# Arktis2022/Spiking-Diffusion

Hardware: AMD Instinct MI355X
Metric: images/sec + LIF-kernel HBM GB/s, MNIST 100-step sample T=16, 1->8 GPU (higher is better)
Workload: dtype fp32-exact (4 fp6 digits x fp4 spikes on the block-scaled MFMA + certified decisions + exact 6-digit recomputation of flagged neurons)

## Files before the change

### spiking-diffusion_amd/csrc/den_mfma_fp6v2.hip

```cpp
#include "cert_common.h"
#include "../../include/spkdiff.h"
#include <stdlib.h>
#include <type_traits>
#include <utility>

namespace {

constexpr int CK = 32;
constexpr int N_PAIR = 18;
constexpr int N_D4 = 5;
constexpr int N_MAIN = N_PAIR + N_D4;
constexpr int N_L5 = 2;
constexpr int NACC = 2;
constexpr int W_PIECES = (N_PAIR * WT + 1023) / 1024;
constexpr int W_LDS = W_PIECES * 1024;
constexpr int W_SLAB = ((N_MAIN + N_L5) * WT + 1023) / 1024 * 1024;

struct V2Args {
  const uint8_t* in0; int nch;
  const uint8_t* wq; const double* scale; const double* bias; const float* wl1;
  const float* bn_a; const float* bn_b;
  uint8_t* out; uint8_t* out_cnt;
  CertWs ws;
  int handover;
  const int* qtab;
  const int* n_dyn;
  const uint8_t* need; const int* cls_cnt; const int* cls_list;
  int B, Cout, Cin;
  int gx, nsets;
};

constexpr int SPK_V2_KMIN = 2;
constexpr float SPK_V2_SPARE = 1.0f;
constexpr int SPK_V2_REC_STEP = 13;
constexpr int SPK_V2_LP_PAIRS = 1;
constexpr int SPK_V2_GX_KB = 2560;
constexpr int SPK_V2_HALF_FILL = 2;
constexpr int SPK_V2_LPS_MIN_B = 64;
constexpr int SPK_V2_LP_SPLIT_MAX = 512;
constexpr int SPK_V2_PF = 6;


__device__ __forceinline__ void store_tile_spikes(uint8_t* out, uint8_t* out_cnt, unsigned mybits, int lane, long long rec_base,
                                                  long long cnt_base, bool ok) {
  const unsigned bitsv = spk_transpose16_rows(mybits, lane);
  if (out_cnt && ok) out_cnt[cnt_base + (lane & 31)] = (uint8_t)__popc(mybits);
  if (ok) *reinterpret_cast<uint2*>(out + rec_base + (lane & 15) * 16 + 8 * ((lane >> 4) & 1)) = spk_e2m1_record(bitsv);
}

__device__ const uint8_t V2_HALF_REC[2][64] = {
    {0, 1, 2, 3, 4, 5, 6, 7, 8, 9, 10, 11, 12, 13, 14, 15, 16, 17, 18, 19, 20, 21, 22, 23,
     23, 23, 23, 23, 23, 23, 23, 23, 23, 23, 23, 23, 23, 23, 23, 23, 23, 23, 23, 23, 23, 23, 23, 23, 24},
    {24, 25, 26, 27, 28, 29, 30, 31, 32, 33, 34, 35, 36, 37, 38, 39, 40, 41, 42, 43, 44, 45, 46, 47,
     47, 47, 47, 47, 47, 47, 47, 47, 47, 47, 47, 47, 47, 47, 47, 47, 47, 47, 47, 47, 47, 47, 47, 47, 24}};

enum : int { V2_INT = 0, V2_TOP, V2_RIGHT, V2_LEFT, V2_BOTTOM, V2_NCLS };
struct V2Plan { int nblk; int tap[9]; int nt[9]; };
constexpr int V2_FT = 3;
constexpr V2Plan V2_PLAN[V2_NCLS] = {
    {9, {0, 1, 2, 3, 4, 5, 6, 7, 8}, {3, 3, 3, 3, 3, 3, 3, 3, 3}},
    {6, {3, 4, 5, 6, 7, 8}, {3, 3, 3, 3, 3, 3}},
    {6, {0, 1, 3, 4, 6, 7}, {3, 3, 3, 3, 3, 3}},
    {6, {1, 2, 4, 5, 7, 8}, {3, 3, 3, 3, 3, 3}},
    {9, {0, 6, 7, 8, 1, 2, 3, 4, 5}, {3, 1, 1, 1, 3, 3, 3, 3, 3}}};
constexpr V2Plan v2_uniform_plan(int nt) {
  V2Plan p = {9, {0, 1, 2, 3, 4, 5, 6, 7, 8}, {}};
  for (int b = 0; b < 9; ++b) p.nt[b] = nt;
  return p;
}
constexpr int v2_plan_start(const V2Plan& p, int blk) {
  int n = 0;
  for (int b = 0; b < blk; ++b) n += p.nt[b];
  return n;
}
constexpr int v2_plan_blk(const V2Plan& p, int s) {
  int b = 0;
  while (s >= p.nt[b]) s -= p.nt[b++];
  return b;
}
__device__ constexpr uint8_t V2_FULL_POS[8][V2_FT][2] = {
    {{0, 1}, {2, 3}, {4, 5}},       {{6, 13}, {20, 27}, {34, 41}},  {{7, 14}, {21, 28}, {35, 42}},  {{43, 44}, {45, 46}, {47, 40}},
    {{8, 9}, {10, 11}, {12, 15}},   {{16, 17}, {18, 19}, {22, 23}}, {{24, 25}, {26, 29}, {30, 31}}, {{32, 33}, {36, 37}, {38, 39}}};
__device__ constexpr uint8_t V2_WAVE_CLS[8] = {V2_TOP, V2_RIGHT, V2_LEFT, V2_BOTTOM, V2_INT, V2_INT, V2_INT, V2_INT};
constexpr bool v2_full_map_ok() {
  bool seen[48] = {};
  for (int w = 0; w < 8; ++w)
    for (int i = 0; i < V2_FT; ++i)
      for (int h = 0; h < 2; ++h) {
        const int p = V2_FULL_POS[w][i][h];
        if (p >= 48 || seen[p]) return false;
        seen[p] = true;
      }
  for (int w = 0; w < 8; ++w) {
    const V2Plan& pl = V2_PLAN[V2_WAVE_CLS[w]];
    for (int i = 0; i < V2_FT; ++i)
      for (int tap = 0; tap < 9; ++tap) {
        int n = 0;
        for (int b = 0; b < pl.nblk; ++b) n += pl.tap[b] == tap && i >= V2_FT - pl.nt[b];
        if (n > 1) return false;
        for (int h = 0; h < 2 && n == 0; ++h) {
          const int y = V2_FULL_POS[w][i][h] / 7 + tap / 3 - 1, x = V2_FULL_POS[w][i][h] % 7 + tap % 3 - 1;
          if (y >= 0 && y < 7 && x >= 0 && x < 7) return false;
        }
      }
  }
  return true;
}
static_assert(v2_full_map_ok(), "full 7x7 items: position table and block lists");

constexpr int V2_FULL_NCA = 3, V2_FULL_NCWW = 3;
constexpr int v2_ceil_div(int a, int b) { return (a + b - 1) / b; }
constexpr int v2_copy_na(int na, int ncw, int w) {
  const int npa = v2_ceil_div(na, ncw), left = na - w * npa;
  return w >= ncw || left <= 0 ? 0 : (left < npa ? left : npa);
}
constexpr int v2_copy_nw(int nw, int ncw, int w) {
  return w >= ncw || w >= nw ? 0 : (nw - w + ncw - 1) / ncw;
}
constexpr int v2_rec_off(int r, int nrec, int w) {
  const int cl = r >> 4, t = r & 15;
  return r < nrec ? (((cl / w) + 1) * (w + 1) + 1 + (cl % w)) * POSB + t * 16 : 0;
}
constexpr bool v2_roles_ok(int nwv, int nca, int ncww, int na, int nw, int nrec, int w) {
  int pa[64] = {}, pw[64] = {};
  if (na > 64 || nw > 64 || nca > nwv || ncww > nwv) return false;
  for (int wv = 0; wv < nwv; ++wv) {
    for (int j = 0; j < v2_copy_na(na, nca, wv); ++j) ++pa[wv * v2_ceil_div(na, nca) + j];
    for (int q = 0; q < v2_copy_nw(nw, ncww, wv); ++q) ++pw[wv + ncww * q];
  }
  for (int i = 0; i < na; ++i) if (pa[i] != 1) return false;
  for (int i = 0; i < nw; ++i) if (pw[i] != 1) return false;
  const int nct = 64 * nwv, nr = v2_ceil_div(nrec, nct);
  int seen[1024] = {};
  if (nrec > 1024) return false;
  for (int tid = 0; tid < nct; ++tid)
    for (int k = 0; k < nr; ++k) {
      const int r = tid + k * nct, off = v2_rec_off(r, nrec, w);
      if (r < nrec) {
        const int cell = off / POSB, y = cell / (w + 1), x = cell % (w + 1);
        if (y < 1 || x < 1 || x > w || (y - 1) * w + (x - 1) != (r >> 4) || (off % POSB) != (r & 15) * 16) return false;
        ++seen[r];
      } else if (off != 0) return false;
    }
  for (int r = 0; r < nrec; ++r) if (seen[r] != 1) return false;
  return true;
}
static_assert(v2_roles_ok(8, V2_FULL_NCA, V2_FULL_NCWW, 7 * 2, W_PIECES, 7 * 7 * 16, 7), "full 7x7 items: 41 pieces, 784 records, one owner each");

template <int H, int W, int NWV, bool SPLIT, int NTP, bool HALF = false, int CLS = V2_INT>
__device__ __forceinline__ void fp6v2_body(const V2Args& a, const int g, const int il, const int lanes, const int n_images,
                                           const int* __restrict__ slots, const int n_live = 0) {
  constexpr bool PRUNE = NTP > 0;
  constexpr bool LIVE = PRUNE && !HALF;
  static_assert(!HALF || (PRUNE && !SPLIT && H == 7 && W == 7 && NWV == 4 && NTP == 3), "half-image items: 7x7, four waves x three tiles");
  constexpr bool REC = !PRUNE;
  constexpr int HW = H * W, PW = W + 1;
  constexpr int Hb = SPLIT ? H / 2 : H;
  constexpr int Hin = SPLIT ? Hb + 1 : H;
  constexpr int HWb = Hb * W;
  static_assert(SPLIT ? ((H % 2) == 0 && (HWb % (2 * NWV)) == 0)
                      : ((HW & 1) == 1 && ((HW / 2) % NWV) == 0), "whole 32-row tiles on every wave (+ one odd position)");
  static_assert(!PRUNE || (!SPLIT && (NWV == 4 || NWV == 8) && NTP <= (HWb / 2) / NWV), "position lists: 7x7 items");
  constexpr int NT = PRUNE ? NTP : (HWb / 2) / NWV;
  constexpr int N_AGPR = NWV == 4 ? (NACC * NT < 16 ? NACC * NT : 16) : 0;
  constexpr int NPP = (Hin + 2) * PW + 1;
  constexpr int A_BYTES = NPP * POSB;
  constexpr int PPR = (W + 3) / 4;
  constexpr int NA = Hin * PPR;
  constexpr bool BSKIP = NWV == 8 && !PRUNE && !SPLIT;
  static_assert(!BSKIP || (H == 7 && W == 7 && NT == V2_FT), "border skip: the position table is for 7x7 items of three tiles per wave");
  static_assert(BSKIP || CLS == V2_INT, "wave classes: full 7x7 items only");
  constexpr int NCA = BSKIP ? V2_FULL_NCA : NWV, NCWW = BSKIP ? V2_FULL_NCWW : NWV;
  constexpr bool KNOWN = BSKIP && CLS != V2_INT;
  constexpr int CWV = KNOWN ? CLS - 1 : 0;
  static_assert(!KNOWN || V2_WAVE_CLS[CWV] == CLS, "border class k is wave k - 1");
  static_assert(!BSKIP || v2_roles_ok(NWV, NCA, NCWW, NA, W_PIECES, Hin * W * 16, W), "copy roles, record counting");
  constexpr int NPA_T = (NA + NCA - 1) / NCA;
  constexpr int NPA = KNOWN ? v2_copy_na(NA, NCA, CWV) : ((!BSKIP || NCA == NWV) ? NPA_T : 0);
  constexpr int NPW = KNOWN ? v2_copy_nw(W_PIECES, NCWW, CWV) : ((!BSKIP || NCWW == NWV) ? (W_PIECES + NCWW - 1) / NCWW : 0);
  static_assert(NWV >= 8 || NACC * NT <= 16 || (NT - 1) * NACC <= N_AGPR + 2, "only the last tile may straddle the register files");
  constexpr bool AH = NWV == 8 && !PRUNE;
  constexpr int NBUF = 2;
  extern __shared__ __attribute__((aligned(16))) uint8_t lds[];
  uint8_t* const sA = lds;
  uint8_t* const sW = lds + NBUF * A_BYTES;
  int* const s_cin = reinterpret_cast<int*>(lds + NBUF * A_BYTES + NBUF * W_LDS);
  int* const s_row = s_cin + NPP * 16;
  int* const s_nmax = s_row + (HWb + 1) * 16;
  const unsigned sA_addr = spk_lds_addr(sA), sW_addr = sA_addr + NBUF * A_BYTES;
  const int tid = threadIdx.x, lane = tid & 63, wave = tid >> 6;
  const int nch = a.nch;
  const int G = a.Cout >> 5;
  const int wave_s = KNOWN ? CWV : __builtin_amdgcn_readfirstlane(wave);
  const unsigned lane16 = (unsigned)lane * 16u;
  const unsigned wave_k = (unsigned)wave_s * 1024u;
  const uint8_t* const wbase = a.wq + (long long)g * nch * W_SLAB;
  const int nitems = (SPLIT || HALF) ? 2 * n_images : n_images;
  auto issue_w = [&](int qw, const uint8_t* wslab, unsigned dW) {
    unsigned ko = wave_k + 1024u * NCWW * (unsigned)qw;
    if (NCWW * qw + NCWW - 1 >= W_PIECES) ko = ko < (unsigned)W_PIECES * 1024u ? ko : ko - 1024u * NCWW;
    spk_dma16s(wslab + ko, lane16, dW + ko);
  };
  if constexpr (BSKIP && NPW > 0) {
    if (il < nitems) {
#pragma unroll
      for (int q = 0; q < NPW; ++q) issue_w(q, wbase, sW_addr);
    }
  }
  for (int i = tid; i < NBUF * A_BYTES / 16; i += NWV * 64) reinterpret_cast<uint4*>(sA)[i] = make_uint4(0, 0, 0, 0);
  if (REC)
    for (int i = tid; i < NPP * 16; i += NWV * 64) s_cin[i] = 0;
  __syncthreads();

  const int row = lane & 31, half = lane >> 5;
  const int hsel = (row >> 2) & 1, tt = (row & 3) + 4 * (row >> 3);
  int a_off[NT];
  int p_out[NT];
#pragma unroll
  for (int i = 0; i < NT; ++i) {
    const int p = BSKIP ? (int)V2_FULL_POS[wave & 7][i % V2_FT][hsel] : 2 * (wave + NWV * i) + hsel;
    a_off[i] = ((p / W) * PW + (p % W)) * POSB + tt * 16;
    p_out[i] = BSKIP ? (int)V2_FULL_POS[wave & 7][i % V2_FT][half] : 2 * (wave + NWV * i) + half;
  }

  unsigned pa_pk[NPA > 0 ? NPA : 1];
#pragma unroll
  for (int j = 0; j < NPA; ++j) {
    int id = wave_s * NPA_T + j;
    id = id < NA ? id : NA - 1;
    const int y = id / PPR, px = id - y * PPR;
    const int np = (W - 4 * px) < 4 ? (W - 4 * px) : 4;
    const unsigned src = (unsigned)((y * W + 4 * px) * POSB), dst = (unsigned)(((y + 1) * PW + 1 + 4 * px) * POSB);
    pa_pk[j] = src | (dst << 14) | ((unsigned)(np - 1) << 29);
  }
  auto issue_piece = [&](int q, const uint8_t* aslab, const uint8_t* wslab, unsigned dA, unsigned dW) {
    if (q < NPA) {
      const unsigned pk = pa_pk[q];
      const unsigned np = ((pk >> 29) & 3u) + 1u;
      const unsigned long long mask = np == 4 ? ~0ull : ((1ull << (16 * np)) - 1ull);
      spk_dma16s_masked(aslab + (pk & 0x3fffu), lane16, dA + ((pk >> 14) & 0x7fffu), mask);
    } else issue_w(q - NPA, wslab, dW);
  };
  auto aslab_of = [&](int itm, int c) -> const uint8_t* {
    const int b = HALF ? itm >> 1 : (PRUNE ? slots[itm] : (SPLIT ? itm >> 1 : itm)), band = SPLIT ? itm & 1 : 0;
    return a.in0 + ((long long)b * nch + c) * HW * POSB + band * (Hb - 1) * W * POSB;
  };

  const int co = g * 32 + (lane & 31);
  const float scale_f = (float)a.scale[co], bias_f = (float)a.bias[co];
  const float bna = a.bn_a[co], bnb = a.bn_b[co];
  const float Bc = fmaf(bias_f, bna, bnb);
  const float cE = 2.0f * 2.38418579e-07f * (fabsf(bnb) + fabsf(Bc)) + 1e-30f;
  const float cT = 528.0f * scale_f * fabsf(bna) * 1.000001f;
  const float Ac4 = 1024.0f * scale_f * bna;

  const int sc_a = 0x7f7f7f7f;
  const int sc_p = half ? (int)0x82828282u : (int)0x87878787u;

  int it = 0;
  if (il < nitems) {
    const uint8_t* as0 = aslab_of(il, 0);
#pragma unroll
    for (int q = 0; q < (BSKIP ? NPA : NPA + NPW); ++q) issue_piece(q, as0, wbase, sA_addr, sW_addr);
    if constexpr (AH) {
      spk_dma_wait_all();
      __syncthreads();
    }
  }
  for (int itm = il; itm < nitems; itm += lanes) {
    const int b = HALF ? itm >> 1 : (PRUNE ? slots[itm] : (SPLIT ? itm >> 1 : itm)), band = SPLIT ? itm & 1 : 0;
    const int band_off = band * PW * POSB;
    int n_list = 2 * NT * NWV;
    if constexpr (PRUNE) {
      const uint8_t* rec = HALF ? &V2_HALF_REC[itm & 1][0] : a.need + (long long)b * 64;
      n_list = __builtin_amdgcn_readfirstlane((int)rec[48]);
#pragma unroll
      for (int i = 0; i < NT; ++i) {
        const int k2 = 2 * (wave + NWV * i);
        const int p = rec[k2 + hsel];
        a_off[i] = ((p / W) * PW + (p % W)) * POSB + tt * 16;
        p_out[i] = rec[k2 + half];
      }
    }
    v16f acc[NT][NACC];
    int cnt[NT];
#pragma unroll
    for (int i = 0; i < NT; ++i) cnt[i] = 0;
    constexpr int NREC = Hin * W * 16, NR = (NREC + NWV * 64 - 1) / (NWV * 64);
    int creg[NR];
    int rec_off[NR];
    bool rec_ok[NR];
#pragma unroll
    for (int k = 0; k < NR; ++k) {
      creg[k] = 0;
      const int r = tid + k * NWV * 64;
      rec_ok[k] = r < NREC;
      rec_off[k] = v2_rec_off(r, NREC, W);
    }
    constexpr int PFX = NWV == 4 ? SPK_V2_PF : 4;
    v6i bp[2][2];
    v4i af[PFX];
    for (int c = 0; c < nch; ++c, ++it) {
      const int buf = it & 1, buf1 = buf ^ 1;
      if constexpr (!AH) {
        spk_dma_wait_all();
        __syncthreads();
      }
      int nb = itm, nc = c + 1;
      if (nc == nch) { nc = 0; nb = itm + lanes; }
      const bool have_next = nb < nitems;
      const uint8_t* n_aslab = aslab_of(have_next ? nb : itm, have_next ? nc : c);
      const uint8_t* n_wslab = wbase + (long long)(have_next ? nc : c) * W_SLAB;
      const unsigned n_dA = sA_addr + buf1 * A_BYTES;
      const unsigned n_dW = sW_addr + buf1 * W_LDS;

      v4i rvq[NR];
      auto compute = [&](auto first_tag) {
        constexpr bool FIRST = decltype(first_tag)::value;
        const uint8_t* A = sA + buf * A_BYTES + band_off;
        const uint8_t* Wb = sW + buf * W_LDS;
        auto toff = [](int tap) constexpr -> int { return ((tap / 3) * PW + (tap % 3)) * POSB; };
        constexpr V2Plan P = BSKIP ? V2_PLAN[CLS] : v2_uniform_plan(NT);
        constexpr int NBLK = P.nblk, NSTEP = v2_plan_start(P, NBLK);
        constexpr int PF = PFX;
        constexpr int NPIECES = NPA + NPW;
        static_assert(P.nt[0] == NT, "the first block writes (not accumulates) every accumulator");
        constexpr bool SLOT1 = BSKIP && (NCA != NWV || NCWW != NWV);
        static_assert(SLOT1 || 2 * NBLK >= NPIECES, "two copy slots per block: every DMA piece of the wave gets one");
        static_assert((!AH || NSTEP >= 2 * PF) && (!REC || NSTEP > SPK_V2_REC_STEP), "look-ahead slots; the record-count steps exist");
        static_assert(!AH || ((SLOT1 ? NPIECES : v2_plan_start(P, (NPIECES + 1) / 2)) <= NSTEP - PF && v2_plan_start(P, NBLK - 2) <= NSTEP - PF),
                      "chunk barrier behind the copies and the last weight-tile read");
        auto lda_at = [&](const uint8_t* base, auto s_tag) -> v4i {
          constexpr int s = decltype(s_tag)::value;
          constexpr int blk = v2_plan_blk(P, s), i = NT - P.nt[blk] + (s - v2_plan_start(P, blk));
          return *reinterpret_cast<const v4i*>(base + a_off[i] + toff(P.tap[blk]));
        };
        auto lda = [&](auto s_tag) -> v4i { return lda_at(A, s_tag); };
        auto ldb = [&](int tile) -> v6i {
          const uint8_t* p = Wb + tile * WT;
          const v4i x = *reinterpret_cast<const v4i*>(p + lane * 16);
          typedef const volatile __attribute__((address_space(3))) v2i* lds_v2i_ptr;
          const v2i y = *(lds_v2i_ptr)SPK_LDS(p + 1024 + lane * 8);
          const v6i r = {x[0], x[1], x[2], x[3], y[0], y[1]};
          return r;
        };
        if constexpr (!AH || FIRST) {
          bp[0][0] = ldb(2 * P.tap[0]); bp[0][1] = ldb(2 * P.tap[0] + 1);
          static_for<PF>([&](auto s_tag) { af[decltype(s_tag)::value] = lda(s_tag); });
        }
        const uint8_t* An = sA + buf1 * A_BYTES + band_off;
        const uint8_t* Wn = sW + buf1 * W_LDS;
        const bool ahead = AH && c + 1 < nch;
        static_for<NSTEP>([&](auto s_tag) {
          constexpr int s = decltype(s_tag)::value;
          constexpr int blk = v2_plan_blk(P, s), nt = P.nt[blk], j = s - v2_plan_start(P, blk);
          constexpr int i = NT - nt + j;
          if constexpr (AH && s == NSTEP - PF) {
            asm volatile("s_waitcnt vmcnt(0)\n\ts_barrier" ::: "memory");
          }
          const v4i av = af[s % PF];
          if constexpr (s + PF < NSTEP) af[s % PF] = lda(std::integral_constant<int, s + PF>{});
          else if constexpr (AH) {
            constexpr int k = s % PF;
            if (ahead) af[k] = lda_at(An, std::integral_constant<int, k>{});
          }
#define V2_DMA_SLOT()                                                                              \
  do {                                                                                             \
    if constexpr (SLOT1 && s < NPIECES) issue_piece(s, n_aslab, n_wslab, n_dA, n_dW);                 \
    if constexpr (!SLOT1 && j == 0 && 2 * blk < NPIECES) issue_piece(2 * blk, n_aslab, n_wslab, n_dA, n_dW);     \
    if constexpr (!SLOT1 && j == (nt > 1 ? nt / 2 : 0) && 2 * blk + 1 < NPIECES)                   \
      issue_piece(2 * blk + 1, n_aslab, n_wslab, n_dA, n_dW);                                      \
  } while (0)
#define V2_NEXT_TILES()                                                                            \
  do {                                                                                             \
    if constexpr (j == 0 && blk + 1 < NBLK) {                                                      \
      bp[(blk + 1) & 1][0] = ldb(2 * P.tap[(blk + 1) % 9]);                                        \
      bp[(blk + 1) & 1][1] = ldb(2 * P.tap[(blk + 1) % 9] + 1);                                    \
    }                                                                                              \
  } while (0)
          if constexpr (!REC) {
            asm volatile("v_bcnt_u32_b32 %0, %1, %0\n\tv_bcnt_u32_b32 %0, %2, %0\n\tv_bcnt_u32_b32 %0, %3, %0\n\t"
                         "v_bcnt_u32_b32 %0, %4, %0" : "+v"(cnt[i]) : "v"(av[0]), "v"(av[1]), "v"(av[2]), "v"(av[3]));
          }
#define V2_PAIR_MFMA(J)                                                                                      \
do {                                                                                                        \
  if constexpr (FIRST && blk == 0) {                                                                        \
    if constexpr (NACC * i + (J) < N_AGPR) SPK_MFMA_FP6_Z("a", acc[i][J], av, bp[0][J], sc_a, sc_p);              \
    else SPK_MFMA_FP6_Z("v", acc[i][J], av, bp[0][J], sc_a, sc_p);                                             \
  } else {                                                                                                  \
    if constexpr (NACC * i + (J) < N_AGPR) SPK_MFMA_FP6("a", acc[i][J], av, bp[blk & 1][J], sc_a, sc_p);          \
    else SPK_MFMA_FP6("v", acc[i][J], av, bp[blk & 1][J], sc_a, sc_p);                                         \
  }                                                                                                         \
} while (0)
          V2_PAIR_MFMA(0);
          __builtin_amdgcn_sched_barrier(0);
          V2_DMA_SLOT();
          V2_NEXT_TILES();
          if constexpr (REC) {
            if constexpr (s == 1) {
#pragma unroll
              for (int k = 0; k < NR; ++k) rvq[k] = *reinterpret_cast<const v4i*>(sA + buf * A_BYTES + rec_off[k]);
            }
            if constexpr (s == SPK_V2_REC_STEP) {
#pragma unroll
              for (int k = 0; k < NR; ++k)
                creg[k] += __builtin_popcount((unsigned)rvq[k][0]) + __builtin_popcount((unsigned)rvq[k][1]) +
                           __builtin_popcount((unsigned)rvq[k][2]) + __builtin_popcount((unsigned)rvq[k][3]);
            }
          }
          V2_PAIR_MFMA(1);
          __builtin_amdgcn_sched_barrier(0);
          if constexpr (AH && s == NSTEP - 1) {
            if (ahead) {
              auto ldb_n = [&](int tile) -> v6i {
                const uint8_t* p = Wn + tile * WT;
                const v4i x = *reinterpret_cast<const v4i*>(p + lane * 16);
                typedef const volatile __attribute__((address_space(3))) v2i* lds_v2i_ptr;
                const v2i y = *(lds_v2i_ptr)SPK_LDS(p + 1024 + lane * 8);
                const v6i r = {x[0], x[1], x[2], x[3], y[0], y[1]};
                return r;
              };
              bp[0][0] = ldb_n(2 * P.tap[0]); bp[0][1] = ldb_n(2 * P.tap[0] + 1);
            }
          }
        });
      };
      if (c == 0) compute(std::true_type{}); else compute(std::false_type{});
    }

    if constexpr (REC) {
#pragma unroll
      for (int k = 0; k < NR; ++k)
        if (rec_ok[k]) s_cin[(rec_off[k] / POSB) * 16 + ((rec_off[k] % POSB) >> 4)] = creg[k];
      if (tid <= HWb) s_nmax[tid] = 0;
      __syncthreads();
      for (int e = tid; e < HWb * 16; e += NWV * 64) {
        const int pp = e >> 4, t = e & 15;
        const int* c0 = s_cin + (((pp / W) + band) * PW + (pp % W)) * 16 + t;
        int sum = 0;
#pragma unroll
        for (int dy = 0; dy < 3; ++dy)
#pragma unroll
          for (int dx = 0; dx < 3; ++dx) sum += c0[(dy * PW + dx) * 16];
        s_row[e] = sum;
        atomicMax(&s_nmax[pp], sum);
      }
      __syncthreads();
    }
    asm volatile("s_nop 15\n\ts_nop 15" ::: "memory");

#pragma unroll
    for (int k = 0; k < NT; ++k) {
      const int i = k == 0 ? NT - 1 : k - 1;
#pragma unroll
      for (int j = 0; j < NACC; ++j)
        if (NACC * i + j < N_AGPR) asm volatile("" : "+a"(acc[i][j]));
      float v = 0.f;
      unsigned mybits = 0;
      bool flg = false;
      int cntv[16];
      if constexpr (!REC) {
#pragma unroll
        for (int r = 0; r < 16; ++r) {
          const int rowA = spk_acc_row(r, 0);
          const int c0 = __builtin_amdgcn_readlane(cnt[i], rowA), c1 = __builtin_amdgcn_readlane(cnt[i], rowA + 4);
          cntv[r] = half ? c1 : c0;
        }
      }
      int nmax_rec = 0;
      if constexpr (REC) nmax_rec = s_nmax[BSKIP ? p_out[i] : 2 * (wave + NWV * i) + half];
      float zmax = 0.f, dmin = 3.0e38f;
      int nmax = nmax_rec;
#pragma unroll
      for (int r2 = 0; r2 < 16; r2 += 2) {
        const v2f p0 = {acc[i][0][r2], acc[i][0][r2 + 1]}, p1 = {acc[i][1][r2], acc[i][1][r2 + 1]};
        const v2f q4 = __builtin_elementwise_fma(p0, (v2f){1024.0f, 1024.0f}, p1);
        const v2f z2 = __builtin_elementwise_fma(q4, (v2f){Ac4, Ac4}, (v2f){Bc, Bc});
        if constexpr (!REC) nmax = max(nmax, max(cntv[r2], cntv[r2 + 1]));
#pragma unroll
        for (int e = 0; e < 2; ++e) {
          const float z = z2[e];
          zmax = fmaxf(zmax, fabsf(z));
          const float h = fmaf(z - v, 0.5f, v);
          const float hm = h - 1.0f;
          dmin = fminf(dmin, fabsf(hm));
          const bool s = h >= 1.0f;
          v = s ? 0.0f : h;
          mybits = __builtin_amdgcn_alignbit(mybits, __float_as_uint(hm), 31);
        }
      }
      mybits = ~(__builtin_bitreverse32(mybits) >> 16) & 0xffffu;
      flg = dmin <= SPK_V2_SPARE * fmaf(zmax, 2.5f * CERT_4EPS, fmaf((float)nmax, cT, cE));
      if (__builtin_amdgcn_ballot_w64(flg) != 0ull) {
        float v2 = 0.f, dh = 0.f;
        bool f2 = false;
        if constexpr (REC) {
          const v4i* rp = reinterpret_cast<const v4i*>(s_row + (BSKIP ? p_out[i] : 2 * (wave + NWV * i) + half) * 16);
#pragma unroll
          for (int q = 0; q < 4; ++q) {
            const v4i c4 = rp[q];
            cntv[4 * q] = c4[0]; cntv[4 * q + 1] = c4[1]; cntv[4 * q + 2] = c4[2]; cntv[4 * q + 3] = c4[3];
          }
        }
#pragma unroll
        for (int r2 = 0; r2 < 16; r2 += 2) {
          const v2f p0 = {acc[i][0][r2], acc[i][0][r2 + 1]}, p1 = {acc[i][1][r2], acc[i][1][r2 + 1]};
          const v2f q4 = __builtin_elementwise_fma(p0, (v2f){1024.0f, 1024.0f}, p1);
          const v2f z2 = __builtin_elementwise_fma(q4, (v2f){Ac4, Ac4}, (v2f){Bc, Bc});
#pragma unroll
          for (int e = 0; e < 2; ++e) {
            const float z = z2[e];
            const float ct = fmaf((float)cntv[r2 + e], cT, cE);
            dh = fmaf(fabsf(z) + fabsf(v2), 0.625f * CERT_4EPS, fmaf(dh, 0.5f, 0.5f * ct));
            const float h = fmaf(z - v2, 0.5f, v2);
            f2 = f2 || (fabsf(h - 1.0f) <= SPK_V2_SPARE * dh);
            v2 = h >= 1.0f ? 0.0f : h;
          }
        }
        flg = flg && f2;
      }
      const int ti = wave + NWV * i;
      const int p = (PRUNE || BSKIP) ? p_out[i] : 2 * ti + half + band * HWb;
      const bool listed = (!PRUNE || 2 * ti + half < n_list) && (!LIVE || b < n_live);
      if (flg && listed) spk_cert_flag(a.ws, ((long long)b * a.Cout + co) * HW + p);
      const long long rec = (((long long)b * G + g) * HW + p) * POSB;
      store_tile_spikes(a.out, a.out_cnt, mybits, lane, rec, (((long long)b * G + g) * HW + p) * 32, listed);
      __builtin_amdgcn_sched_barrier(0);
    }
  }
  spk_dma_wait_all();
}

__device__ __forceinline__ void fp6v2_wg_map(const V2Args& a, int& g, int& il, int& lanes) {
  const int k = blockIdx.x, G = a.Cout >> 5;
  if (a.gx > 0) {
    const int S = gridDim.x >> 3, x = k & 7, slot = k >> 3;
    const int npart = 8 / a.nsets, set = x % a.nsets, xi = x / a.nsets, lanes_x = S / a.gx;
    g = set * a.gx + slot % a.gx;
    il = xi * lanes_x + slot / a.gx;
    lanes = npart * lanes_x;
  } else {
    g = k % G;
    il = k / G;
    lanes = gridDim.x / G;
  }
}

__device__ __forceinline__ void fp6v2_handover(const V2Args& a) {
  if (!a.handover) return;
  __syncthreads();
  if (threadIdx.x == 0) spk_cert_handover(a.ws);
}

template <int H, int W, int NWV, bool SPLIT = false>
__global__ __launch_bounds__(NWV * 64, 1) void conv3x3_fp6v2_kernel(V2Args a) {
  const int Bn = spk_batch_count(a.n_dyn, a.B);
  int g, il, lanes;
  fp6v2_wg_map(a, g, il, lanes);
  if constexpr (NWV == 8 && !SPLIT) {
    switch (__builtin_amdgcn_readfirstlane((int)V2_WAVE_CLS[(threadIdx.x >> 6) & 7])) {
      case V2_TOP: fp6v2_body<H, W, NWV, false, 0, false, V2_TOP>(a, g, il, lanes, Bn, nullptr); break;
      case V2_RIGHT: fp6v2_body<H, W, NWV, false, 0, false, V2_RIGHT>(a, g, il, lanes, Bn, nullptr); break;
      case V2_LEFT: fp6v2_body<H, W, NWV, false, 0, false, V2_LEFT>(a, g, il, lanes, Bn, nullptr); break;
      case V2_BOTTOM: fp6v2_body<H, W, NWV, false, 0, false, V2_BOTTOM>(a, g, il, lanes, Bn, nullptr); break;
      default: fp6v2_body<H, W, NWV, false, 0, false, V2_INT>(a, g, il, lanes, Bn, nullptr); break;
    }
  } else fp6v2_body<H, W, NWV, SPLIT, 0>(a, g, il, lanes, Bn, nullptr);
  fp6v2_handover(a);
}

template <int H, int W>
__global__ __launch_bounds__(256, 1) void conv3x3_fp6v2_half_kernel(V2Args a) {
  const int Bn = spk_batch_count(a.n_dyn, a.B);
  int g, il, lanes;
  fp6v2_wg_map(a, g, il, lanes);
  fp6v2_body<H, W, 4, false, 3, true>(a, g, il, lanes, Bn, nullptr);
  fp6v2_handover(a);
}

template <int H, int W, int NWV>
__global__ __launch_bounds__(NWV * 64, 1) void conv3x3_fp6v2_listed_kernel(V2Args a) {
  constexpr int NC = (H * W / 2) / 4;
  const int Bn = spk_batch_count(a.n_dyn, a.B);
  int g, il, lanes;
  fp6v2_wg_map(a, g, il, lanes);
  int cnt[NC], work[NC], u[NC];
  int total = 0, nonempty = 0;
#pragma unroll
  for (int k = 0; k < NC; ++k) {
    cnt[k] = a.cls_cnt[k];
    work[k] = cnt[k] * (k + 1 < SPK_V2_KMIN ? SPK_V2_KMIN : k + 1);
    total += work[k];
    nonempty += cnt[k] > 0;
  }
  if (total == 0) { fp6v2_handover(a); return; }
  int rem = lanes - nonempty, used = 0;
#pragma unroll
  for (int k = 0; k < NC; ++k) {
    u[k] = cnt[k] > 0 ? 1 + (int)((long long)rem * work[k] / total) : 0;
    used += u[k];
  }
  for (int left = lanes - used; left > 0; --left) {
    int best = 0;
    long long bw = -1, bu = 1;
#pragma unroll
    for (int k = 0; k < NC; ++k)
      if (cnt[k] > 0 && (long long)work[k] * bu > bw * u[k]) { bw = work[k]; bu = u[k]; best = k; }
#pragma unroll
    for (int k = 0; k < NC; ++k) u[k] += (k == best);
  }
  int start = 0, cls = -1, il_c = 0, lanes_c = 1;
#pragma unroll
  for (int k = 0; k < NC; ++k) {
    if (il >= start && il < start + u[k]) { cls = k; il_c = il - start; lanes_c = u[k]; }
    start += u[k];
  }
  const int* slots = a.cls_list + (long long)(cls < 0 ? 0 : cls) * a.B;
  static_assert(NWV == 8, "listed positions: two waves per SIMD");
  switch (cls) {
    case 0: case 1: fp6v2_body<H, W, 8, false, 1>(a, g, il_c, lanes_c, cnt[cls], slots, Bn); break;
    case 2: case 3: fp6v2_body<H, W, 8, false, 2>(a, g, il_c, lanes_c, cnt[cls], slots, Bn); break;
    case 4: case 5: fp6v2_body<H, W, 8, false, 3>(a, g, il_c, lanes_c, cnt[cls], slots, Bn); break;
    default: break;
  }
  fp6v2_handover(a);
}


template <int H, int W, bool WIDE>
__device__ __forceinline__ void fp6v2_lastpos_body(const V2Args& a, const int bid, float (*red)[16][64]) {
  constexpr int HW = H * W, NP = SPK_V2_LP_PAIRS;
  const int lane = threadIdx.x & 63, wave = threadIdx.x >> 6;
  const int nch = a.nch, G = a.Cout >> 5;
  const int Bn = spk_batch_count(a.n_dyn, a.B);
  if (!a.handover && bid == 0 && threadIdx.x == 0) { a.ws.flags[1] = a.ws.flags[0]; a.ws.flags[0] = 0u; }
  const int n_units = ((Bn + 2 * NP - 1) / (2 * NP)) * G;
  const bool split = n_units <= SPK_V2_LP_SPLIT_MAX;
  const int unit = split ? bid : bid * 4 + wave;
  const int g = unit % G, b0 = (unit / G) * 2 * NP;
  if (b0 >= Bn) return;
  const int row = lane & 31, half = lane >> 5;
  const int hsel = (row >> 2) & 1, tt = (row & 3) + 4 * (row >> 3);
  const int sc_a = 0x7f7f7f7f;
  const int sc_p = half ? (int)0x82828282u : (int)0x87878787u;
  const int sc_hi = (int)0x87878787u, sc_lo = (int)0x82828282u;
  v16f acc[NP][3];
#pragma unroll
  for (int q = 0; q < NP; ++q)
#pragma unroll
    for (int j = 0; j < 3; ++j)
#pragma unroll
      for (int r = 0; r < 16; ++r) acc[q][j][r] = 0.f;
  const int py = H - 1, px = W - 1;
  for (int c = split ? wave : 0; c < nch; c += split ? 4 : 1) {
    const uint8_t* wslab = a.wq + ((long long)g * nch + c) * W_SLAB;
    auto ldb = [&](int tile) -> v8i {
      const uint8_t* wt = wslab + tile * WT;
      const v4i bx = *reinterpret_cast<const v4i*>(wt + lane * 16);
      const v2i by = *reinterpret_cast<const v2i*>(wt + 1024 + lane * 8);
      return v8i{bx[0], bx[1], bx[2], bx[3], by[0], by[1], 0, 0};
    };
    v4i sp[NP][4];
#pragma unroll
    for (int q = 0; q < NP; ++q) {
      const int bA = b0 + 2 * q + hsel;
#pragma unroll
      for (int u = 0; u < 4; ++u) {
        const int tap = (u >> 1) * 3 + (u & 1);
        const int yy = py + tap / 3 - 1, xx = px + tap % 3 - 1;
        sp[q][u] = v4i{0, 0, 0, 0};
        if (bA < Bn)
          sp[q][u] = *reinterpret_cast<const v4i*>(a.in0 + (((long long)bA * nch + c) * HW + yy * W + xx) * POSB + tt * 16);
      }
// ... 454 lines not shown
```

Before: 3361.

## Pair adjacent conv taps per MFMA block with compile-time register-slot schedule

For the block-skip (full 7x7) path, adjacent 3x3 taps are grouped into pair blocks so each block covers two taps. The two half-waves read different tap offsets and the weight tiles use interleaved high/low scale selectors, which roughly halves the number of block iterations. A constexpr scheduler places each A and B LDS read a fixed distance ahead of its MFMA, bounded by when its register slot frees up and by the chunk barrier, and static_asserts check that placement. DMA pieces and record-count ops are moved into fixed slots. This adds heavy template complexity and changes register pressure and the scale encoding, which could break exactness if the pairing is wrong.

```diff
diff --git a/spiking-diffusion_amd/csrc/den_mfma_fp6v2.hip b/spiking-diffusion_amd/csrc/den_mfma_fp6v2.hip
--- a/spiking-diffusion_amd/csrc/den_mfma_fp6v2.hip
+++ b/spiking-diffusion_amd/csrc/den_mfma_fp6v2.hip
@@ -39,6 +39,10 @@
 constexpr int SPK_V2_LPS_MIN_B = 64;
 constexpr int SPK_V2_LP_SPLIT_MAX = 512;
 constexpr int SPK_V2_PF = 6;
+constexpr int SPK_V2_TP_SLOTS_INT = 5;
+constexpr int v2_tp_slots(int cls) { return cls == 0 ? SPK_V2_TP_SLOTS_INT : (cls == 4 ? 4 : 3); }
+constexpr int SPK_V2_TP_PFD = 12;
+constexpr int SPK_V2_TP_TAIL = 6;
 
 
 __device__ __forceinline__ void store_tile_spikes(uint8_t* out, uint8_t* out_cnt, unsigned mybits, int lane, long long rec_base,
@@ -55,16 +59,16 @@
      47, 47, 47, 47, 47, 47, 47, 47, 47, 47, 47, 47, 47, 47, 47, 47, 47, 47, 47, 47, 47, 47, 47, 47, 24}};
 
 enum : int { V2_INT = 0, V2_TOP, V2_RIGHT, V2_LEFT, V2_BOTTOM, V2_NCLS };
-struct V2Plan { int nblk; int tap[9]; int nt[9]; };
+struct V2Plan { int nblk; int tap[9]; int nt[9]; int pair[9]; };
 constexpr int V2_FT = 3;
 constexpr V2Plan V2_PLAN[V2_NCLS] = {
-    {9, {0, 1, 2, 3, 4, 5, 6, 7, 8}, {3, 3, 3, 3, 3, 3, 3, 3, 3}},
-    {6, {3, 4, 5, 6, 7, 8}, {3, 3, 3, 3, 3, 3}},
-    {6, {0, 1, 3, 4, 6, 7}, {3, 3, 3, 3, 3, 3}},
-    {6, {1, 2, 4, 5, 7, 8}, {3, 3, 3, 3, 3, 3}},
-    {9, {0, 6, 7, 8, 1, 2, 3, 4, 5}, {3, 1, 1, 1, 3, 3, 3, 3, 3}}};
+    {5, {0, 2, 4, 6, 8}, {3, 3, 3, 3, 3}, {1, 1, 1, 1, 0}},
+    {3, {3, 5, 7}, {3, 3, 3}, {1, 1, 1}},
+    {3, {0, 3, 6}, {3, 3, 3}, {1, 1, 1}},
+    {3, {1, 4, 7}, {3, 3, 3}, {1, 1, 1}},
+    {5, {0, 6, 8, 2, 4}, {3, 1, 1, 3, 3}, {1, 1, 0, 1, 1}}};
 constexpr V2Plan v2_uniform_plan(int nt) {
-  V2Plan p = {9, {0, 1, 2, 3, 4, 5, 6, 7, 8}, {}};
+  V2Plan p = {9, {0, 1, 2, 3, 4, 5, 6, 7, 8}, {}, {}};
   for (int b = 0; b < 9; ++b) p.nt[b] = nt;
   return p;
 }
@@ -77,6 +81,73 @@
   int b = 0;
   while (s >= p.nt[b]) s -= p.nt[b++];
   return b;
+}
+constexpr bool v2_plan_has(const V2Plan& p, int b, int tap) { return p.tap[b] == tap || (p.pair[b] && p.tap[b] + 1 == tap); }
+constexpr int v2p_nd(const V2Plan& p, int b) { return p.pair[b] ? 4 : 2; }
+constexpr int v2p_op_start(const V2Plan& p, int blk) {
+  int n = 0;
+  for (int b = 0; b < blk; ++b) n += v2p_nd(p, b) * p.nt[b];
+  return n;
+}
+constexpr int v2p_op_blk(const V2Plan& p, int m) {
+  int b = 0;
+  while (m >= v2p_op_start(p, b + 1)) ++b;
+  return b;
+}
+constexpr int v2p_swap(int q) { return ((q & 1) << 1) | (q >> 1); }
+constexpr int v2p_op_sel(const V2Plan& p, int b, int q) { return p.nt[b] > 1 ? q / p.nt[b] : (p.pair[b] ? v2p_swap(q) : q); }
+constexpr int v2p_op_tile(const V2Plan& p, int b, int q) { return V2_FT - p.nt[b] + (p.nt[b] > 1 ? q % p.nt[b] : 0); }
+constexpr int v2p_b_start(const V2Plan& p, int blk) {
+  int n = 0;
+  for (int b = 0; b < blk; ++b) n += v2p_nd(p, b);
+  return n;
+}
+constexpr int v2p_b_blk(const V2Plan& p, int g) {
+  int b = 0;
+  while (g >= v2p_b_start(p, b + 1)) ++b;
+  return b;
+}
+constexpr int v2p_a_first(const V2Plan& p, int f) { return v2p_op_start(p, v2_plan_blk(p, f)) + f - v2_plan_start(p, v2_plan_blk(p, f)); }
+constexpr int v2p_a_last(const V2Plan& p, int f) { return v2p_a_first(p, f) + (v2p_nd(p, v2_plan_blk(p, f)) - 1) * p.nt[v2_plan_blk(p, f)]; }
+constexpr int v2p_b_first(const V2Plan& p, int g) {
+  const int b = v2p_b_blk(p, g), sel = g - v2p_b_start(p, b);
+  return v2p_op_start(p, b) + (p.nt[b] > 1 ? sel * p.nt[b] : (p.pair[b] ? v2p_swap(sel) : sel));
+}
+constexpr int v2p_b_last(const V2Plan& p, int g) { return v2p_b_first(p, g) + p.nt[v2p_b_blk(p, g)] - 1; }
+struct V2Sched { int nf, nb, nm, mb; int a_at[27]; int b_at[36]; int a_dist, b_dist; bool ok; };
+constexpr V2Sched v2p_sched(const V2Plan& p, int nslot, int pfd, int tail) {
+  V2Sched s = {};
+  s.nf = v2_plan_start(p, p.nblk); s.nb = v2p_b_start(p, p.nblk); s.nm = v2p_op_start(p, p.nblk); s.mb = s.nm - tail;
+  s.ok = s.nf <= 27 && s.nb <= 36 && s.nf >= nslot && tail > 0 && s.mb > 0;
+  s.a_dist = s.b_dist = s.nm;
+  for (int f = 0; f < s.nf && s.ok; ++f) {
+    int free_at = -s.nm;
+    for (int k = 1; k <= s.nf; ++k) {
+      const int g = f - k, gg = g < 0 ? g + s.nf : g;
+      if (gg % nslot == f % nslot) { free_at = v2p_a_last(p, gg) + 1 - (g < 0 ? s.nm : 0); break; }
+    }
+    const int first = v2p_a_first(p, f);
+    int at = free_at > first - pfd ? free_at : first - pfd;
+    if (at < 0 && at < s.mb - s.nm) at = s.mb - s.nm;
+    s.a_at[f] = at;
+    s.a_dist = first - at < s.a_dist ? first - at : s.a_dist;
+    s.ok = s.ok && at >= free_at && at <= first && (at < 0 ? at + s.nm >= s.mb : at <= s.mb);
+  }
+  for (int g = 0; g < s.nb && s.ok; ++g) {
+    const int sel = g - v2p_b_start(p, v2p_b_blk(p, g));
+    int free_at = -s.nm;
+    for (int k = 1; k <= s.nb; ++k) {
+      const int h = g - k, hh = h < 0 ? h + s.nb : h;
+      if (hh - v2p_b_start(p, v2p_b_blk(p, hh)) == sel) { free_at = v2p_b_last(p, hh) + 1 - (h < 0 ? s.nm : 0); break; }
+    }
+    const int first = v2p_b_first(p, g);
+    int at = free_at;
+    if (at < 0 && at < s.mb - s.nm) at = s.mb - s.nm;
+    s.b_at[g] = at;
+    s.b_dist = first - at < s.b_dist ? first - at : s.b_dist;
+    s.ok = s.ok && at >= free_at && at <= first && (at < 0 ? at + s.nm >= s.mb : at <= s.mb);
+  }
+  return s;
 }
 __device__ constexpr uint8_t V2_FULL_POS[8][V2_FT][2] = {
     {{0, 1}, {2, 3}, {4, 5}},       {{6, 13}, {20, 27}, {34, 41}},  {{7, 14}, {21, 28}, {35, 42}},  {{43, 44}, {45, 46}, {47, 40}},
@@ -91,20 +162,24 @@
         if (p >= 48 || seen[p]) return false;
         seen[p] = true;
       }
+  int steps = 0;
   for (int w = 0; w < 8; ++w) {
     const V2Plan& pl = V2_PLAN[V2_WAVE_CLS[w]];
+    for (int b = 0; b < pl.nblk; ++b)
+      if (pl.tap[b] + pl.pair[b] > 8 || pl.nt[b] < 1 || pl.nt[b] > V2_FT) return false;
     for (int i = 0; i < V2_FT; ++i)
       for (int tap = 0; tap < 9; ++tap) {
         int n = 0;
-        for (int b = 0; b < pl.nblk; ++b) n += pl.tap[b] == tap && i >= V2_FT - pl.nt[b];
+        for (int b = 0; b < pl.nblk; ++b) n += v2_plan_has(pl, b, tap) && i >= V2_FT - pl.nt[b];
         if (n > 1) return false;
+        steps += n;
         for (int h = 0; h < 2 && n == 0; ++h) {
           const int y = V2_FULL_POS[w][i][h] / 7 + tap / 3 - 1, x = V2_FULL_POS[w][i][h] % 7 + tap % 3 - 1;
           if (y >= 0 && y < 7 && x >= 0 && x < 7) return false;
         }
       }
   }
-  return true;
+  return steps == 11 * 6 + 13 * 9;
 }
 static_assert(v2_full_map_ok(), "full 7x7 items: position table and block lists");
 
@@ -213,6 +288,8 @@
   __syncthreads();
 
   const int row = lane & 31, half = lane >> 5;
+  const int a_hd1 = half * POSB, a_hd2 = half * (PW - 2) * POSB;
+  const int b_o16 = lane * 16 + half * (2 * WT - 512), b_o8 = 1024 + lane * 8 + half * (2 * WT - 256);
   const int hsel = (row >> 2) & 1, tt = (row & 3) + 4 * (row >> 3);
   int a_off[NT];
   int p_out[NT];
@@ -256,6 +333,7 @@
 
   const int sc_a = 0x7f7f7f7f;
   const int sc_p = half ? (int)0x82828282u : (int)0x87878787u;
+  const int sc_hi = (int)0x87878787u, sc_lo = (int)0x82828282u;
 
   int it = 0;
   if (il < nitems) {
@@ -297,7 +375,7 @@
       rec_ok[k] = r < NREC;
       rec_off[k] = v2_rec_off(r, NREC, W);
     }
-    constexpr int PFX = NWV == 4 ? SPK_V2_PF : 4;
+    constexpr int PFX = BSKIP ? v2_tp_slots(CLS) : (NWV == 4 ? SPK_V2_PF : 4);
     v6i bp[2][2];
     v4i af[PFX];
     for (int c = 0; c < nch; ++c, ++it) {
@@ -315,20 +393,112 @@
       const unsigned n_dW = sW_addr + buf1 * W_LDS;
 
       v4i rvq[NR];
+      auto compute_tap_pairs = [&](auto first_tag, const uint8_t* A, const uint8_t* Wb) {
+        constexpr bool FIRST = decltype(first_tag)::value;
+        constexpr V2Plan P = V2_PLAN[BSKIP ? CLS : V2_INT];
+        constexpr V2Sched S = v2p_sched(P, PFX, SPK_V2_TP_PFD, SPK_V2_TP_TAIL);
+        constexpr int NM = S.nm, MB = S.mb, NF = S.nf, NB = S.nb, NPIECES = NPA + NPW;
+        static_assert(S.ok, "tap pairs: every read in front of its first use, behind its register set's last use, on the right side of the chunk barrier");
+        static_assert(S.a_dist >= 2 && S.b_dist >= (CLS == V2_BOTTOM ? 1 : 3), "no read right in front of the MFMA that needs it");
+        static_assert(P.pair[0] && P.nt[0] == NT, "the first block writes (not accumulates) every accumulator: digits 0 and 2 of a pair block");
+        static_assert((NPIECES == 0 || 2 * (NPIECES - 1) < MB) && 2 * SPK_V2_REC_STEP < MB, "copy slots and record-count ops in front of the chunk barrier");
+        auto toff = [](int tap) constexpr -> int { return ((tap / 3) * PW + (tap % 3)) * POSB; };
+        auto lda = [&](const uint8_t* base, auto f_tag) -> v4i {
+          constexpr int f = decltype(f_tag)::value, blk = v2_plan_blk(P, f), i = NT - P.nt[blk] + (f - v2_plan_start(P, blk));
+          constexpr int t0 = toff(P.tap[blk]), dl = P.pair[blk] ? toff(P.tap[blk] + 1) - t0 : 0;
+          static_assert(dl == 0 || dl == POSB || dl == (PW - 2) * POSB, "a pair's second tap: the next cell, or the first of the next row");
+          const int o = dl == 0 ? a_off[i] : a_off[i] + (dl == POSB ? a_hd1 : a_hd2);
+          return *reinterpret_cast<const v4i*>(base + o + t0);
+        };
+        auto ldb = [&](const uint8_t* base, auto g_tag) -> v6i {
+          constexpr int g = decltype(g_tag)::value, blk = v2p_b_blk(P, g), sel = g - v2p_b_start(P, blk);
+          constexpr int tile = 2 * P.tap[blk] + (P.pair[blk] ? sel >> 1 : sel), odd = P.pair[blk] ? sel & 1 : 0;
+          const uint8_t* p = base + tile * WT;
+          const int o16 = P.pair[blk] ? b_o16 + 512 * odd : lane * 16, o8 = P.pair[blk] ? b_o8 + 256 * odd : 1024 + lane * 8;
+          const v4i x = *reinterpret_cast<const v4i*>(p + o16);
+          typedef const volatile __attribute__((address_space(3))) v2i* lds_v2i_ptr;
+          const v2i y = *(lds_v2i_ptr)SPK_LDS(p + o8);
+          const v6i r = {x[0], x[1], x[2], x[3], y[0], y[1]};
+          return r;
+        };
+        if constexpr (FIRST) {
+          static_for<NB>([&](auto g_tag) {
+            constexpr int g = decltype(g_tag)::value, sel = g - v2p_b_start(P, v2p_b_blk(P, g));
+            if constexpr (S.b_at[g] < 0) bp[sel >> 1][sel & 1] = ldb(Wb, g_tag);
+          });
+          static_for<NF>([&](auto f_tag) {
+            constexpr int f = decltype(f_tag)::value;
+            if constexpr (S.a_at[f] < 0) af[f % PFX] = lda(A, f_tag);
+          });
+        }
+        const uint8_t* An = sA + buf1 * A_BYTES + band_off;
+        const uint8_t* Wn = sW + buf1 * W_LDS;
+        const bool ahead = c + 1 < nch;
+        static_for<NM>([&](auto m_tag) {
+          constexpr int m = decltype(m_tag)::value, blk = v2p_op_blk(P, m), q = m - v2p_op_start(P, blk);
+          constexpr int sel = v2p_op_sel(P, blk, q), i = v2p_op_tile(P, blk, q);
+          constexpr int f = v2_plan_start(P, blk) + i - (NT - P.nt[blk]);
+          static_for<NB>([&](auto g_tag) {
+            constexpr int g = decltype(g_tag)::value, gs = g - v2p_b_start(P, v2p_b_blk(P, g));
+            if constexpr (S.b_at[g] == m) bp[gs >> 1][gs & 1] = ldb(Wb, g_tag);
+          });
+          static_for<NF>([&](auto f_tag) {
+            if constexpr (S.a_at[decltype(f_tag)::value] == m) af[decltype(f_tag)::value % PFX] = lda(A, f_tag);
+          });
+          if constexpr (m == MB) {
+            asm volatile("s_waitcnt vmcnt(0)\n\ts_barrier" ::: "memory");
+          }
+          if constexpr (m >= MB) {
+            if (ahead) {
+              static_for<NB>([&](auto g_tag) {
+                constexpr int g = decltype(g_tag)::value, gs = g - v2p_b_start(P, v2p_b_blk(P, g));
+                if constexpr (S.b_at[g] + NM == m) bp[gs >> 1][gs & 1] = ldb(Wn, g_tag);
+              });
+              static_for<NF>([&](auto f_tag) {
+                if constexpr (S.a_at[decltype(f_tag)::value] + NM == m) af[decltype(f_tag)::value % PFX] = lda(An, f_tag);
+              });
+            }
+          }
+          if constexpr (!P.pair[blk]) {
+            SPK_MFMA_FP6("v", acc[i][sel], af[f % PFX], bp[0][sel], sc_a, sc_p);
+          } else if constexpr (FIRST && blk == 0 && (sel & 1) == 0) {
+            SPK_MFMA_FP6_Z("v", acc[i][sel >> 1], af[f % PFX], bp[sel >> 1][0], sc_a, sc_hi);
+          } else if constexpr ((sel & 1) == 0) {
+            SPK_MFMA_FP6("v", acc[i][sel >> 1], af[f % PFX], bp[sel >> 1][0], sc_a, sc_hi);
+          } else {
+            SPK_MFMA_FP6("v", acc[i][sel >> 1], af[f % PFX], bp[sel >> 1][1], sc_a, sc_lo);
+          }
+          __builtin_amdgcn_sched_barrier(0);
+          if constexpr ((m & 1) == 0 && m / 2 < NPIECES) issue_piece(m / 2, n_aslab, n_wslab, n_dA, n_dW);
+          if constexpr (m == 2) {
+#pragma unroll
+            for (int k = 0; k < NR; ++k) rvq[k] = *reinterpret_cast<const v4i*>(sA + buf * A_BYTES + rec_off[k]);
+          }
+          if constexpr (m == 2 * SPK_V2_REC_STEP) {
+#pragma unroll
+            for (int k = 0; k < NR; ++k)
+              creg[k] += __builtin_popcount((unsigned)rvq[k][0]) + __builtin_popcount((unsigned)rvq[k][1]) +
+                         __builtin_popcount((unsigned)rvq[k][2]) + __builtin_popcount((unsigned)rvq[k][3]);
+          }
+        });
+      };
       auto compute = [&](auto first_tag) {
         constexpr bool FIRST = decltype(first_tag)::value;
         const uint8_t* A = sA + buf * A_BYTES + band_off;
         const uint8_t* Wb = sW + buf * W_LDS;
         auto toff = [](int tap) constexpr -> int { return ((tap / 3) * PW + (tap % 3)) * POSB; };
-        constexpr V2Plan P = BSKIP ? V2_PLAN[CLS] : v2_uniform_plan(NT);
+        if constexpr (BSKIP) {
+          compute_tap_pairs(first_tag, A, Wb);
+          return;
+        }
+        constexpr V2Plan P = v2_uniform_plan(NT);
         constexpr int NBLK = P.nblk, NSTEP = v2_plan_start(P, NBLK);
         constexpr int PF = PFX;
         constexpr int NPIECES = NPA + NPW;
         static_assert(P.nt[0] == NT, "the first block writes (not accumulates) every accumulator");
-        constexpr bool SLOT1 = BSKIP && (NCA != NWV || NCWW != NWV);
-        static_assert(SLOT1 || 2 * NBLK >= NPIECES, "two copy slots per block: every DMA piece of the wave gets one");
+        static_assert(2 * NBLK >= NPIECES, "two copy slots per block: every DMA piece of the wave gets one");
         static_assert((!AH || NSTEP >= 2 * PF) && (!REC || NSTEP > SPK_V2_REC_STEP), "look-ahead slots; the record-count steps exist");
-        static_assert(!AH || ((SLOT1 ? NPIECES : v2_plan_start(P, (NPIECES + 1) / 2)) <= NSTEP - PF && v2_plan_start(P, NBLK - 2) <= NSTEP - PF),
+        static_assert(!AH || (v2_plan_start(P, (NPIECES + 1) / 2) <= NSTEP - PF && v2_plan_start(P, NBLK - 2) <= NSTEP - PF),
                       "chunk barrier behind the copies and the last weight-tile read");
         auto lda_at = [&](const uint8_t* base, auto s_tag) -> v4i {
           constexpr int s = decltype(s_tag)::value;
@@ -366,9 +536,8 @@
           }
 #define V2_DMA_SLOT()                                                                              \
   do {                                                                                             \
-    if constexpr (SLOT1 && s < NPIECES) issue_piece(s, n_aslab, n_wslab, n_dA, n_dW);                 \
-    if constexpr (!SLOT1 && j == 0 && 2 * blk < NPIECES) issue_piece(2 * blk, n_aslab, n_wslab, n_dA, n_dW);     \
-    if constexpr (!SLOT1 && j == (nt > 1 ? nt / 2 : 0) && 2 * blk + 1 < NPIECES)                   \
+    if constexpr (j == 0 && 2 * blk < NPIECES) issue_piece(2 * blk, n_aslab, n_wslab, n_dA, n_dW);                \
+    if constexpr (j == (nt > 1 ? nt / 2 : 0) && 2 * blk + 1 < NPIECES)                             \
       issue_piece(2 * blk + 1, n_aslab, n_wslab, n_dA, n_dW);                                      \
   } while (0)
 #define V2_NEXT_TILES()                                                                            \
```

Result: faster. 3433, median of 6 (+2.2%).
